# Labbeti/conette-audio-captioning

Hardware: AMD Instinct MI355X
Metric: clips_per_sec (higher is better)
Workload: dtype bf16; 1 GPU; B=64/GPU x 10 s @ 32 kHz clips, ConvNeXt encoder + beam-3 KV-cached decode (min 3 / max 20 tokens, V=5631), synthetic seeded checkpoint; batch_per_gpu=64, global_batch=64, beam_size=3, parallelism=dp1, world_size_observed=1, allreduce_of_ones=1, decode_group=2, decode_streams=2, encode_streams=1, input_batches_rotated=4

## Files before the change

conette-audio-captioning_amd/csrc/api.hip:

```cpp
#include <math.h>
#include <stdarg.h>
#include <stdlib.h>

#include <string>
#include <unordered_map>
#include <vector>

#include "ctx.h"
#include <algorithm>
#include "mlp_rc2.h"
#include "mlp_rs.h"
#include "mlp_rs16.h"
#include "mlp_sp.h"
#include "down_fused.h"

static thread_local char g_err[512] = "";

void cn_set_error(const char* fmt, ...) {
  va_list ap;
  va_start(ap, fmt);
  vsnprintf(g_err, sizeof(g_err), fmt, ap);
  va_end(ap);
}

extern "C" const char* conette_last_error(void) { return g_err; }

struct CnProfRec {
  int cls;
  hipEvent_t start, stop;
};
struct CnRuntime {
  std::vector<CnProfRec> recs;
  std::vector<hipEvent_t> free_ev;
  int open_cls = -1;
  hipEvent_t open_start = nullptr;
};

static hipEvent_t rt_event(CnRuntime* rt) {
  if (!rt->free_ev.empty()) {
    hipEvent_t e = rt->free_ev.back();
    rt->free_ev.pop_back();
    return e;
  }
  hipEvent_t e = nullptr;
  (void)hipEventCreate(&e);
  return e;
}

void cn_prof_begin(conette_ctx* ctx, int cls, hipStream_t s) {
  CnRuntime* rt = ctx->rt;
  rt->open_cls = cls;
  rt->open_start = rt_event(rt);
  (void)hipEventRecord(rt->open_start, s);
}
void cn_prof_end(conette_ctx* ctx, int cls, hipStream_t s) {
  CnRuntime* rt = ctx->rt;
  if (rt->open_cls != cls || !rt->open_start) return;
  hipEvent_t stop = rt_event(rt);
  (void)hipEventRecord(stop, s);
  rt->recs.push_back(CnProfRec{cls, rt->open_start, stop});
  rt->open_cls = -1;
  rt->open_start = nullptr;
}
// ... 150 lines not shown
    const float* src = find(name, n);
    if (n < 0) n = 0;
    float* dst = (float*)alloc((size_t)n * 4);
    if (src) hipLaunchKernelGGL((pk_copy<float>), dim3(256), dim3(256), 0, 0, src, dst, (size_t)n);
    return dst;
  }
  const void* operand(const std::string& name, int64_t total, int64_t first, int64_t n) {
    const float* src = find(name, total);
    void* dst = alloc((size_t)n * ctx->esize);
    if (src) {
      copy_operand(src + first, dst, (size_t)n);
    }
    return dst;
  }
  void copy_operand(const float* src, void* dst, size_t n) {
    if (ctx->esize == 2) CN_H16_CALL(ctx, hipLaunchKernelGGL((pk_copy<HT>), dim3(256), dim3(256), 0, 0, src, (HT*)dst, n));
    else if (ctx->sp16) hipLaunchKernelGGL((pk_copy<sp16_t>), dim3(256), dim3(256), 0, 0, src, (sp16_t*)dst, n);
    else hipLaunchKernelGGL((pk_copy<float>), dim3(256), dim3(256), 0, 0, src, (float*)dst, n);
  }
};

extern "C" int conette_create(const conette_config* cfg, int32_t n_tensors, const char* const* names,
                              const void* const* tensors, const int64_t* numel, conette_ctx** out) {
  if (!cfg || !names || !tensors || !numel || !out || n_tensors <= 0) {
    cn_set_error("create: bad argument");
    return CN_ERR_ARG;
  }
  if (cfg->precision != CONETTE_PREC_F32 && cfg->precision != CONETTE_PREC_BF16 && cfg->precision != CONETTE_PREC_F16X2 &&
      cfg->precision != CONETTE_PREC_F16) {
    cn_set_error(cfg->precision == 3 ? "create: precision 3 (the experimental fp8 mode of ABI 2) was withdrawn in ABI 3: e4m3 operands cost the "
                                       "frame embeddings 4 %% whatever the scaling (profiles/r06_notes.md section 3)"
                                     : "create: unknown precision %d", cfg->precision);
    return CN_ERR_ARG;
  }
  if (cfg->n_layers < 1 || cfg->n_layers > CN_MAX_LAYERS || cfg->d_model != 256 || cfg->nhead != 8 ||
      cfg->d_ff % 32 != 0 || cfg->vocab_size < 4) {
    cn_set_error("create: unsupported decoder geometry (d_model=%d nhead=%d layers=%d d_ff=%d)", cfg->d_model,
                 cfg->nhead, cfg->n_layers, cfg->d_ff);
    return CN_ERR_ARG;
  }
  conette_ctx* ctx = new conette_ctx();
  memset(ctx, 0, sizeof(*ctx));
  ctx->cfg = *cfg;
  ctx->rt = new CnRuntime();
  ctx->esize = (cfg->precision == CONETTE_PREC_BF16 || cfg->precision == CONETTE_PREC_F16) ? 2 : 4;
  ctx->f16 = cfg->precision == CONETTE_PREC_F16 ? 1 : 0;
  ctx->sp16 = cfg->precision == CONETTE_PREC_F16X2 ? 1 : 0;
  {
    int dev = 0, n_cu = 0;
    if (hipGetDevice(&dev) != hipSuccess || hipDeviceGetAttribute(&n_cu, hipDeviceAttributeMultiprocessorCount, dev) != hipSuccess ||
        n_cu <= 0)
      n_cu = 256;
    ctx->n_cu = n_cu;
  }
  size_t total = (1 << 20) + (size_t)CN_N_BINS * CN_N_MELS * 4;
  for (int i = 0; i < n_tensors; ++i) total += cn_align((size_t)numel[i] * 4) + 256;
  if (cfg->precision == CONETTE_PREC_F16X2) {
    total += 8u << 20;
    total += (size_t)cfg->n_layers * ((size_t)12 * 131072 + (size_t)(cfg->d_ff / 256 + 1) * 4 * 131072 + 4096);
  }
  ctx->arena_bytes = total;
  hipError_t e = hipMalloc((void**)&ctx->arena, total);
  if (e != hipSuccess) {
    cn_set_error("create: hipMalloc(%zu) -> %s", total, hipGetErrorString(e));
    delete ctx->rt;
    delete ctx;
    return CN_ERR_HIP;
  }
  Builder B;
  B.ctx = ctx;
  B.tensors = tensors;
  B.numel = numel;
  for (int i = 0; i < n_tensors; ++i) B.index[names[i]] = i;
  const int d = cfg->d_model, V = cfg->vocab_size, dff = cfg->d_ff;
  const std::string E = "preprocessor.encoder.";
  bool has_encoder = false;
  for (int i = 0; i < n_tensors && !has_encoder; ++i) has_encoder = strncmp(names[i], E.c_str(), E.size()) == 0;
  ctx->no_encoder = has_encoder ? 0 : 1;

  if (has_encoder) {
  {
    const float* cr = B.find(E + "spectrogram_extractor.stft.conv_real.weight", (int64_t)CN_N_BINS * CN_N_FFT);
    float* win = (float*)B.alloc(CN_N_FFT * 4);
    if (cr) hipMemcpy(win, cr, CN_N_FFT * 4, hipMemcpyDeviceToDevice);
    ctx->window = win;
    const float* ci = B.find(E + "spectrogram_extractor.stft.conv_imag.weight", (int64_t)CN_N_BINS * CN_N_FFT);
    if (cr && ci && B.err == CN_OK) {
      const int rows[5] = {1, 7, 100, 333, 512};
      std::vector<float> hw(CN_N_FFT), hr(CN_N_FFT), hi(CN_N_FFT);
      hipMemcpy(hw.data(), cr, CN_N_FFT * 4, hipMemcpyDeviceToHost);
      float wmax = 0.f;
      for (float v : hw) wmax = fmaxf(wmax, fabsf(v));
      double worst = 0.0;
      for (int k : rows) {
        hipMemcpy(hr.data(), cr + (size_t)k * CN_N_FFT, CN_N_FFT * 4, hipMemcpyDeviceToHost);
        hipMemcpy(hi.data(), ci + (size_t)k * CN_N_FFT, CN_N_FFT * 4, hipMemcpyDeviceToHost);
        for (int n = 0; n < CN_N_FFT; n += 13) {
          const double a = -2.0 * M_PI * (double)((long)k * n % CN_N_FFT) / CN_N_FFT;
          worst = fmax(worst, fabs(hr[n] - hw[n] * cos(a)));
          worst = fmax(worst, fabs(hi[n] - hw[n] * sin(a)));
        }
      }
      if (!(wmax > 0.f) || worst > 1e-4 * wmax) {
        cn_set_error("create: spectrogram_extractor.stft.conv_real / conv_imag are not a windowed DFT (max deviation %.3g of "
                     "window peak %.3g): the FFT frontend cannot reproduce this checkpoint", worst, (double)wmax);
        B.err = CN_ERR_WEIGHT;
// ... 389 lines not shown
```

conette-audio-captioning_amd/csrc/ctx.h:

```cpp
#pragma once
#include "../../include/conette_hip.h"
#include "common.h"

#define CN_N_MELS 224
#define CN_N_FFT 1024
#define CN_HOP 320
#define CN_N_BINS 513
#define CN_N_TAGS 527
#define CN_FEAT 768
#define CN_MAX_LAYERS 12

static const int CN_DEPTHS[4] = {3, 3, 9, 3};
static const int CN_DIMS[4] = {96, 192, 384, 768};

struct CnBlockW {
  const float* dw_w;
  const unsigned* dw_wp;
  const float* dw_b;
  const float* ln_w;
  const float* ln_b;
  const void* w1;
  const float* b1;
  const void* w2;
  const float* b2;
// ... 21 lines not shown
  const float* ca_out_b;
  const void* ff1_w;
  const float* ff1_b;
  const void* ff2_w;
  const float* ff2_b;
  const float *n1w, *n1b, *n2w, *n2b, *n3w, *n3b;
  const void* blk_w;
  const void* ffn_w;
  const float* blk_p;
};

struct CnRuntime;

struct conette_ctx {
  conette_config cfg;
  CnRuntime* rt;
  void* dec_graphs;
  uint32_t prof_mask;
  int dec_unfused;
  int esize;
  int sp16;
  int f16;
  int no_encoder;
  const float* window;
  const float2* tw512;
  const float2* tw1024;
  const int* band;
  int mel_rows;
  const float* melC;
  const float* bn_scale;
  const float* bn_shift;
  const float* stem_w;
  const float* stem_b;
  const float* stem_ln_w;
  const float* stem_ln_b;
  CnBlockW blocks[18];
  CnDownW down[3];
  const float* norm_w;
  const float* norm_b;
  const void* head_w;
  const float* head_b;
  const void* proj_w;
  const float* proj_b;
  const void* kv_w;
  const float* kv_b;
  CnLayerW layers[CN_MAX_LAYERS];
  const float* emb;
  const float* pe;
  int pe_len;
  const void* cls_w;
  const float* cls_b;
  int n_cu;
  int enc_reserved_cus;
  int forcing_stepwise;
  char* arena;
  size_t arena_bytes;
  size_t arena_used;
};

void cn_prof_begin(conette_ctx* ctx, int cls, hipStream_t s);
void cn_prof_end(conette_ctx* ctx, int cls, hipStream_t s);
struct CnProfScope {
  conette_ctx* ctx;
  int cls;
  hipStream_t s;
  CnProfScope(conette_ctx* c, int k, hipStream_t st) : ctx(c), cls(k), s(st) {
    if (ctx->prof_mask & (1u << cls)) cn_prof_begin(ctx, cls, s);
  }
  ~CnProfScope() {
    if (ctx->prof_mask & (1u << cls)) cn_prof_end(ctx, cls, s);
  }
};

int cn_frontend(conette_ctx* ctx, const float* wave, int B, int L, float* out, hipStream_t s);

#define CN_BY_PRECISION(ctx, ...)                                                          \
  do {                                                                                     \
    switch ((ctx)->cfg.precision) {                                                        \
      case CONETTE_PREC_BF16: { typedef bf16_t OT; return __VA_ARGS__; }                   \
      case CONETTE_PREC_F16: { typedef half_t OT; return __VA_ARGS__; }                    \
      case CONETTE_PREC_F16X2: { typedef sp16_t OT; return __VA_ARGS__; }                  \
      default: { typedef float OT; return __VA_ARGS__; }                                   \
    }                                                                                      \
  } while (0)
#define CN_H16_CALL(ctx, ...)                          \
  do {                                                 \
    if ((ctx)->f16) { typedef half_t HT; __VA_ARGS__; } \
    else { typedef bf16_t HT; __VA_ARGS__; }            \
  } while (0)
```

conette-audio-captioning_amd/csrc/encoder.hip:

```cpp
#include <stddef.h>

#include "ctx.h"
#include <type_traits>

__device__ int g_cn_nonfinite;
__device__ __forceinline__ void cn_watch_stat(float v) {
  if (!(__builtin_fabsf(v) <= 3.0e38f)) atomicAdd(&g_cn_nonfinite, 1);
}

#include "gemm2.h"
#include "mlp_rc2.h"
#include "mlp_rs.h"
#include "mlp_rs16.h"
#include "mlp_sp.h"
#include "down_fused.h"

#ifndef CN_DW_DOT2
#define CN_DW_DOT2 1
#endif

template <int P, typename XT>
__global__ __launch_bounds__(256) void cn_stem_kernel(const float* __restrict__ in, int F, int H0, long n_pos,
                                                      const float* __restrict__ w ,
                                                      const float* __restrict__ bias, const float* __restrict__ ln_w,
                                                      const float* __restrict__ ln_b, XT* __restrict__ out) {
  __shared__ __attribute__((aligned(16))) float s_w[16 * 96];
  __shared__ __attribute__((aligned(16))) float s_o[P * 64 * 96];
  for (int i = threadIdx.x; i < 16 * 96; i += 256) s_w[i] = w[i];
  __syncthreads();
  const int q = threadIdx.x & 3, lp = threadIdx.x >> 2;
  const long pos0 = (long)blockIdx.x * (64 * P);
  float xin[P][16];
#pragma unroll
  for (int u = 0; u < P; ++u) {
    const long pos = pos0 + 64 * u + lp;
    const long p = pos < n_pos ? pos : n_pos - 1;
    const int wq = (int)(p % 56);
    const long t = p / 56;
    const int h = (int)(t % H0);
    const int b = (int)(t / H0);
#pragma unroll
    for (int i = 0; i < 4; ++i) {
      const int r = 4 * h - 4 + i;
      f32x4 v = {0.f, 0.f, 0.f, 0.f};
      if (r >= 0 && r < F) v = *(const f32x4*)(in + ((size_t)b * F + r) * CN_N_MELS + 4 * wq);
      xin[u][4 * i] = v[0], xin[u][4 * i + 1] = v[1], xin[u][4 * i + 2] = v[2], xin[u][4 * i + 3] = v[3];
    }
  }
  f32x4 acc[P][6];
#pragma unroll
  for (int j = 0; j < 6; ++j) {
    const f32x4 b4 = *(const f32x4*)(bias + q * 24 + 4 * j);
#pragma unroll
    for (int u = 0; u < P; ++u) acc[u][j] = b4;
  }
#pragma unroll
  for (int i = 0; i < 16; ++i)
#pragma unroll
    for (int j = 0; j < 6; ++j) {
      const f32x4 w4 = *(const f32x4*)(s_w + i * 96 + q * 24 + 4 * j);
#pragma unroll
      for (int u = 0; u < P; ++u) acc[u][j] += xin[u][i] * w4;
    }
#pragma unroll
// ... 910 lines not shown
    const int C = CN_DIMS[st], H = g.H[st], W = g.W[st];
    const long P = (long)B * H * W;
    if (st > 0) {
      const int Cp = CN_DIMS[st - 1], Hp = g.H[st - 1], Wp = g.W[st - 1];
      const long n_in = (long)B * Hp * Wp;
      const CnDownW& dw = ctx->down[st - 1];
      CnProfScope ps(ctx, CONETTE_PROF_DOWNSAMPLE, s);
      bool fused_down = false;
      if constexpr (CnIsH16<T>::value) if (Cp <= 192 && dw.fused != nullptr) {
        XT* xo = xc == wsx ? (XT*)ws.h : wsx;
        const int nb = ctx->n_cu - ctx->enc_reserved_cus;
        if (Cp == 96) CN_TRY((cn_launch_down_fused<96, 8, T, XT>(xc, B, Hp, Wp, dw.fused, xo, nb, s)));
        else CN_TRY((cn_launch_down_fused_ring<192, 4, 4, 3, T, XT>(xc, B, Hp, Wp, dw.fused, xo, nb, s)));
        xc = xo;
        if (taps) CN_TRY(tap_copy(taps->down[st], xc, (size_t)P * C, s));
        fused_down = true;
      }
      if (!fused_down) {
      const int ppb = Cp == 96 ? 32 : 16;
      const dim3 pg((unsigned)((n_in + ppb - 1) / ppb));
      if (Cp == 96)
        hipLaunchKernelGGL((cn_ln_patchify_kernel<T, XT, 96>), pg, dim3(256), 0, s, xc, Hp, Wp, n_in, dw.ln_w, dw.ln_b, y);
      else if (Cp == 192)
        hipLaunchKernelGGL((cn_ln_patchify_kernel<T, XT, 192>), pg, dim3(256), 0, s, xc, Hp, Wp, n_in, dw.ln_w, dw.ln_b, y);
      else
        hipLaunchKernelGGL((cn_ln_patchify_kernel<T, XT, 384>), pg, dim3(256), 0, s, xc, Hp, Wp, n_in, dw.ln_w, dw.ln_b, y);
      CN_LAUNCH_CHECK();
      EpiBiasAct<XT, ACT_NONE> epi{dw.bias, wsx, C, ACT_NONE};
      CN_TRY(cn_mm(y, 4 * Cp, (const T*)dw.w, 4 * Cp, (int)P, C, 4 * Cp, epi, s));
      xc = wsx;
      if (taps) CN_TRY(tap_copy(taps->down[st], xc, (size_t)P * C, s));
      }
    }
    for (int b = 0; b < CN_DEPTHS[st]; ++b, ++blk) {
      const CnBlockW& bw = ctx->blocks[blk];
      {
        CnProfScope ps(ctx, CONETTE_PROF_DWCONV_LN, s);
        CN_TRY((dwconv_dispatch<T, XT>(C, xc, B, H, W, bw, y, s)));
      }
      bool fused = false;
      if constexpr (std::is_same<T, sp16_t>::value) {
        if (bw.mlp_sp != nullptr && C <= 192) {
          CnProfScope ps(ctx, CONETTE_PROF_PW1_GEMM, s);
          const int nb = ctx->n_cu - ctx->enc_reserved_cus;
          if (C == 96) CN_TRY((cn_launch_mlp_sp_ring<96, CN_SP_NW96, CN_SP_NST96>(y, bw.mlp_sp, xc, (int)P, nb, s)));
          else CN_TRY((cn_launch_mlp_sp_ring<192, 8, 3>(y, bw.mlp_sp, xc, (int)P, nb, s)));
          fused = true;
        }
      }
      if constexpr (CnIsH16<T>::value) if (!fused) {
        if (bw.mlp_stream != nullptr && C <= 384) {
          CnProfScope ps(ctx, CONETTE_PROF_PW1_GEMM, s);
          const T* wsm = (const T*)bw.mlp_stream;
          if (C == 96) CN_TRY((cn_launch_mlp_rc2_resident<96, 12, 1>(y, wsm, xc, (int)P, ctx->n_cu - ctx->enc_reserved_cus, s)));
          else if (C == 192) CN_TRY((cn_launch_mlp_rc2_ring<192, 8, CN_RC2_NCK(192), CN_RC2_NCK(192) == 2 ? 3 : 5>(y, wsm, xc, (int)P, ctx->n_cu - ctx->enc_reserved_cus, s)));
#ifdef CN_NO_RS
          else CN_TRY((cn_launch_mlp_rc2_ring<384, 4, 1, 3>(y, wsm, xc, (int)P, ctx->n_cu - ctx->enc_reserved_cus, s)));
#else
          else if constexpr (sizeof(XT) == 2 && CN_RS16) CN_TRY((cn_launch_mlp_rs16<384, 4, 3, CN_RS_PRIO>(y, wsm, xc, (int)P, ctx->n_cu - ctx->enc_reserved_cus, s)));
          else CN_TRY((cn_launch_mlp_rs<384, 4, 3, CN_RS_PRIO>(y, wsm, xc, (int)P, ctx->n_cu - ctx->enc_reserved_cus, s)));
#endif
          fused = true;
        }
      }
      if (!fused) {
        {
          CnProfScope ps(ctx, CONETTE_PROF_PW1_GEMM, s);
#ifdef CN_G2_NOACT
          constexpr int kAct = ACT_NONE;
#else
          constexpr int kAct = CnGeluAct<T>::value;
#endif
          EpiBiasAct<T, kAct> e1{bw.b1, hbuf, 4 * C, kAct};
          CN_TRY(cn_mm(y, C, (const T*)bw.w1, C, (int)P, 4 * C, C, e1, s));
        }
        {
          CnProfScope ps(ctx, CONETTE_PROF_PW2_GEMM, s);
          EpiResidT<XT> e2{bw.b2, bw.scale, xc, xc, C};
          CN_TRY(cn_mm(hbuf, 4 * C, (const T*)bw.w2, 4 * C, (int)P, C, 4 * C, e2, s));
        }
      }
      if (taps && b == 0) CN_TRY(tap_copy(taps->stage_block0[st], xc, (size_t)P * C, s));
      if (taps && taps->struct_bytes >= offsetof(conette_encode_taps, block) + (size_t)(blk + 1) * sizeof(float*))
        CN_TRY(tap_copy(taps->block[blk], xc, (size_t)P * C, s));
    }
    if (taps) CN_TRY(tap_copy(taps->stage[st], xc, (size_t)P * C, s));
  }
  const int Tn = g.H[3];
  CnProfScope ps_heads(ctx, CONETTE_PROF_HEADS, s);
  hipLaunchKernelGGL((cn_frame_mean_kernel<T, XT>), dim3((unsigned)(B * Tn)), dim3(256), 0, s, xc, g.W[3], CN_FEAT,
                     frame_embs, (T*)nullptr);
  CN_LAUNCH_CHECK();
  if (clip_probs) {
    hipLaunchKernelGGL((cn_clip_pool_ln_kernel<T>), dim3((unsigned)B), dim3(256), 0, s, frame_embs, Tn, ctx->norm_w,
                       ctx->norm_b, (T*)ws.clip_t);
    CN_LAUNCH_CHECK();
    EpiBiasAct<float> eh{ctx->head_b, clip_probs, CN_N_TAGS, ACT_SIGMOID};
    CN_TRY(cn_mm((const T*)ws.clip_t, CN_FEAT, (const T*)ctx->head_w, CN_FEAT, B, CN_N_TAGS, CN_FEAT, eh, s));
  }
  return CN_OK;
}

extern "C" int conette_encode_nonfinite(conette_ctx* ctx, void* stream, int32_t* count) {
  if (!ctx || !count) {
    cn_set_error("encode_nonfinite: bad argument");
    return CN_ERR_ARG;
  }
// ... 65 lines not shown
```

conette-audio-captioning_amd/csrc/mlp_rc2.h:

```cpp
#pragma once
#include "common.h"

template <int C, int NCK> struct Rc2Geom {
  static constexpr int KS1 = C / 16, NT2 = C / 32, NCH = C / 8;
  static constexpr int F1 = KS1 + 1, F2 = 2 * NT2;
  static constexpr int NSTEP = NCH / NCK;
  static constexpr int FRAGS = NCK * (F1 + F2);
  static constexpr int STEP_BYTES = FRAGS * 1024;
  static constexpr size_t STREAM_BYTES = (size_t)NSTEP * STEP_BYTES;
  static constexpr size_t TOTAL_BYTES = STREAM_BYTES + NT2 * 1024;
};
__host__ __device__ constexpr int cn_rc2_chan(int m) { return (m & 19) | ((m & 4) << 1) | ((m & 8) >> 1); }

__device__ __forceinline__ float cn_gelu_sig2(float x) {
  constexpr float L2E = 1.4426950408889634f;
  const float x2 = fminf(x * x, 64.0f);
  float p = fmaf(x2, 0.0007030350670982541f * L2E, -0.07401130190658815f * L2E);
  p = fmaf(p, x2, -1.5950157568571721f * L2E);
  const float e = __builtin_amdgcn_exp2f(x * p);
  return x * __builtin_amdgcn_rcpf(1.0f + e);
}

#if defined(CN_GELU_SIG2)
#define CN_MLP_XSCALE 1.0f
// ... 25 lines not shown
static __global__ void pk_mlp_rc2(const float* __restrict__ W1, const float* __restrict__ b1, const float* __restrict__ W2,
                           const float* __restrict__ b2, const float* __restrict__ scale, int C, int NCK,
                           HT* __restrict__ dst) {
  const int KS1 = C / 16, NT2 = C / 32, NCH = C / 8, F1 = KS1 + 1, F2 = 2 * NT2, FRAGS = NCK * (F1 + F2), NSTEP = NCH / NCK;
  const int u = blockIdx.x * blockDim.x + threadIdx.x;
  if (u >= (NSTEP * FRAGS + NT2) * 64) return;
  const int l = u & 63, q = (u >> 6) % FRAGS, st = (u >> 6) / FRAGS;
  const int r = l & 31, h = l >> 5;
  float v[8];
  if (st >= NSTEP) {
    const int c = 32 * q + cn_rc2_chan(r);
    const float b = scale[c] * b2[c];
    const float hi = (float)(HT)b;
#pragma unroll
    for (int i = 0; i < 8; ++i) v[i] = 0.f;
    if (h == 0) {
      v[0] = hi;
      v[1] = b - hi;
    }
  } else if (q < NCK * F1) {
    const int j = st * NCK + q / F1, s = q % F1;
    if (s < KS1) {
#pragma unroll
      for (int i = 0; i < 8; ++i) v[i] = CN_MLP_XSCALE * W1[(size_t)(32 * j + r) * C + 16 * s + 8 * h + i];
    } else {
      const float b = CN_MLP_XSCALE * b1[32 * j + r];
      const float hi = (float)(HT)b;
#pragma unroll
      for (int i = 0; i < 8; ++i) v[i] = 0.f;
      if (h == 0) {
        v[0] = hi;
        v[1] = b - hi;
      }
    }
  } else {
    const int q2 = q - NCK * F1;
    const int j = st * NCK + q2 / F2, s = (q2 % F2) / NT2, t = (q2 % F2) % NT2;
    const int c = 32 * t + cn_rc2_chan(r);
    const float sc = scale[c];
#pragma unroll
    for (int i = 0; i < 8; ++i) v[i] = sc * W2[(size_t)c * (4 * C) + 32 * j + 16 * s + 8 * (i >> 2) + 4 * h + (i & 3)];
  }
#pragma unroll
  for (int i = 0; i < 8; ++i) dst[(size_t)u * 8 + i] = (HT)v[i];
}

#define CN_RC2_NCK(C) ((C) == 192 ? 2 : 1)

#define CN_SG_VALU 0x002
#define CN_SG_MFMA 0x008
#define CN_SG_DSR 0x100


template <int C, int NCK, typename HT = bf16_t, typename XT = float> struct Rc2Wave {
  typedef Rc2Geom<C, NCK> G;
  typedef cn_h8<HT> hx8;
  static constexpr int KS1 = G::KS1, NT2 = G::NT2, F1 = G::F1, F2 = G::F2;
  static constexpr int NV = 88;

  static __device__ __forceinline__ hx8 frag(const char* wc, int f) { return *(const hx8*)(wc + f * 1024); }
  static __device__ __forceinline__ f32x16 mma(hx8 a, hx8 b, f32x16 c) { return cn_mma32(a, b, c); }
  static __device__ __forceinline__ hx8 gelu8(const f32x16& X, int o) {
    float g[8];
#pragma unroll
    for (int i = 0; i < 8; ++i) g[i] = cn_gelu_mlp<HT>(X[o + i]);
    return cn_sat8<HT>(cn_pack8<HT>(g[0], g[1], g[2], g[3], g[4], g[5], g[6], g[7]));
  }
  static __device__ __forceinline__ f32x16 zero16() {
    f32x16 z;
#pragma unroll
    for (int i = 0; i < 16; ++i) z[i] = 0.f;
    return z;
  }

  static constexpr int PRE = 4;
  static constexpr int NM = NCK * (F1 + F2), R = PRE + 1;
  struct State {
    hx8 F[R];
    f32x16 X[NCK];
    float g[NCK][16];
    hx8 H[NCK][2];
  };
  static constexpr int gelu_at(int i, int e) {
    if (NCK == 2) return i == 0 ? F1 + 1 + e * (F1 - 1) / 16 : 2 * F1 + e * F2 / 16;
    return e < 8 ? F1 - 1 : F1 + (e - 8) * NT2 / 8;
  }
  template <int Q, int I, int E>
  static __device__ __forceinline__ void gelu_slices(State& st) {
#if defined(CN_RC2_GELU_PK) && defined(CN_GELU_SIG2)
    if constexpr ((E & 1) == 0 && gelu_at(I, E) == Q) {
      const f32x2 r = cn_gelu_sig2_pk(f32x2{st.X[I][E], st.X[I][E + 1]});
      st.g[I][E] = r[0];
      st.g[I][E + 1] = r[1];
    }
    if constexpr (gelu_at(I, E & ~1) == Q) {
#else
    if constexpr (gelu_at(I, E) == Q) {
      st.g[I][E] = cn_gelu_mlp<HT>(st.X[I][E]);
#endif
      if constexpr ((E & 7) == 7) {
        constexpr int o = E - 7;
        st.H[I][E >> 3] = cn_sat8<HT>(cn_pack8<HT>(st.g[I][o], st.g[I][o + 1], st.g[I][o + 2], st.g[I][o + 3],
                                                   st.g[I][o + 4], st.g[I][o + 5], st.g[I][o + 6], st.g[I][o + 7]));
      }
    }
    if constexpr (E + 1 < 16) gelu_slices<Q, I, E + 1>(st);
    else if constexpr (I + 1 < NCK) gelu_slices<Q, I + 1, 0>(st);
  }
  template <int Q>
  static __device__ __forceinline__ void mstep(const char* wc, const hx8 (&fy)[KS1], const hx8 ones, f32x16 (&O)[NT2],
                                               State& st) {
    if constexpr (Q + PRE < NM) st.F[(Q + PRE) % R] = frag(wc, Q + PRE);
    if constexpr (Q < NCK * F1) {
      constexpr int i = Q / F1, s = Q % F1;
      if constexpr (s == 0) st.X[i] = zero16();
      if constexpr (s < KS1) st.X[i] = mma(st.F[Q % R], fy[s], st.X[i]);
      else st.X[i] = mma(st.F[Q % R], ones, st.X[i]);
    } else {
      constexpr int q2 = Q - NCK * F1, i = q2 / F2, k = (q2 % F2) / NT2, t = q2 % NT2;
      O[t] = mma(st.F[Q % R], st.H[i][k], O[t]);
    }
    gelu_slices<Q, 0, 0>(st);
    __builtin_amdgcn_sched_barrier(0);
    if constexpr (Q + 1 < NM) mstep<Q + 1>(wc, fy, ones, O, st);
  }
  template <int Q>
  static __device__ __forceinline__ void prefetch(const char* wc, State& st) {
    st.F[Q % R] = frag(wc, Q);
    if constexpr (Q + 1 < PRE) prefetch<Q + 1>(wc, st);
  }
  static __device__ __forceinline__ void step(const char* wc, const hx8 (&fy)[KS1], const hx8 ones, f32x16 (&O)[NT2]) {
    State st;
    prefetch<0>(wc, st);
    __builtin_amdgcn_sched_barrier(0);
    mstep<0>(wc, fy, ones, O, st);
  }


  static __device__ __forceinline__ void load_y(const HT* __restrict__ Y, int m0, int lane, hx8 (&fy)[KS1]) {
    const HT* base = Y + (size_t)m0 * C;
    const int voff = (lane & 31) * C + 8 * (lane >> 5);
#pragma unroll
    for (int s = 0; s < KS1; ++s) fy[s] = *(const hx8*)(base + voff + 16 * s);
  }

  static __device__ __forceinline__ void init_o(const XT* __restrict__ X, const char* __restrict__ bbf, const hx8 ones, int m0,
                                                int lane, f32x16 (&O)[NT2]) {
    const XT* base = X + (size_t)m0 * C;
    const int voff = (lane & 31) * C + 8 * (lane >> 5);
    hx8 fb[NT2];
    if constexpr (sizeof(XT) == 2) {
      cn_h8<XT> v[NT2][2];
#pragma unroll
      for (int t = 0; t < NT2; ++t) {
        v[t][0] = *(const cn_h8<XT>*)(base + voff + 32 * t);
        v[t][1] = *(const cn_h8<XT>*)(base + voff + 32 * t + 16);
      }
#pragma unroll
// ... 28 lines not shown
#pragma unroll
        for (int o = 0; o < 2; ++o)
          *(cn_h8<XT>*)(base + voff + 32 * t + 16 * o) = cn_pack8<XT>(O[t][8 * o], O[t][8 * o + 1], O[t][8 * o + 2], O[t][8 * o + 3],
                                                                      O[t][8 * o + 4], O[t][8 * o + 5], O[t][8 * o + 6], O[t][8 * o + 7]);
      } else {
#pragma unroll
        for (int q = 0; q < 4; ++q)
          *(f32x4*)(base + voff + 32 * t + 16 * (q >> 1) + 4 * (q & 1)) = f32x4{O[t][4 * q], O[t][4 * q + 1], O[t][4 * q + 2], O[t][4 * q + 3]};
      }
    }
  }
};

template <int C> struct Rc2IoCl {
  static constexpr int NT2 = C / 32;
  static __device__ __forceinline__ void init_o(const float* __restrict__ X, int m0, int lane, f32x16 (&O)[NT2]) {
    const int voff = 4 * (lane >> 5) * C + (lane & 31);
#pragma unroll
    for (int r = 0; r < 16; ++r) {
      const float* row = X + (size_t)(m0 + (r & 3) + 8 * (r >> 2)) * C;
#pragma unroll
      for (int t = 0; t < NT2; ++t) O[t][r] = row[voff + 32 * t];
    }
  }
  static __device__ __forceinline__ void store_o(float* __restrict__ X, const float* __restrict__ bbv, int m0, int M, int lane,
                                                 const f32x16 (&O)[NT2]) {
    const int voff = 4 * (lane >> 5) * C + (lane & 31);
    const int plim = M - m0 - 4 * (lane >> 5);
    float bb[NT2];
#pragma unroll
    for (int t = 0; t < NT2; ++t) bb[t] = bbv[32 * t + (lane & 31)];
#pragma unroll
    for (int r = 0; r < 16; ++r) {
      float* row = X + (size_t)(m0 + (r & 3) + 8 * (r >> 2)) * C;
      if ((r & 3) + 8 * (r >> 2) < plim) {
#pragma unroll
        for (int t = 0; t < NT2; ++t) row[voff + 32 * t] = O[t][r] + bb[t];
      }
    }
  }
};

static inline int cn_rc2_grid(int n_tiles, int waves_per_block, int max_blocks) {
  const int block_tiles = cn_cdiv(n_tiles, waves_per_block);
  if (max_blocks < 1) max_blocks = 1;
  const int rounds = cn_cdiv(block_tiles, max_blocks);
  return cn_cdiv(block_tiles, rounds);
}

template <int C, int NW, int NCK, typename HT = bf16_t, int ABL = 0, typename XT = float>
__global__ __launch_bounds__(NW * 64) void cn_mlp_rc2_resident_kernel(const HT* __restrict__ Y, const HT* __restrict__ WS,
                                                                      XT* __restrict__ X, int M) {
  typedef Rc2Geom<C, NCK> G;
  typedef Rc2Wave<C, NCK, HT, XT> W;
  typedef cn_h8<HT> hx8;
  extern __shared__ __attribute__((aligned(16))) char smem[];
  const int tid = threadIdx.x, lane = tid & 63;
  const int wave = __builtin_amdgcn_readfirstlane(tid >> 6);
  constexpr int TOTAL = G::NSTEP * G::FRAGS;
  for (int i = wave; i < TOTAL; i += NW)
    __builtin_amdgcn_global_load_lds((const __attribute__((address_space(1))) void*)((const char*)WS + (size_t)i * 1024 + lane * 16),
                                     (__attribute__((address_space(3))) void*)(smem + i * 1024), 16, 0, 0);
  const char* bbf = (const char*)WS + G::STREAM_BYTES + lane * 16;
  const int n_tiles = (M + 31) >> 5;
  const int t_lo = (int)((long)blockIdx.x * n_tiles / gridDim.x), t_hi = (int)((long)(blockIdx.x + 1) * n_tiles / gridDim.x);
  hx8 ones;
#pragma unroll
  for (int i = 0; i < 8; ++i) ones[i] = (HT)((lane < 32 && i < 2) ? 1.0f : 0.0f);
  hx8 fy[G::KS1];
  int tile = t_lo + wave;
  if (tile < t_hi) W::load_y(Y, tile * 32, lane, fy);
  asm volatile("s_waitcnt vmcnt(0)" ::: "memory");
  __syncthreads();
  const char* wl = smem + lane * 16;
  for (; tile < t_hi; tile += NW) {
    f32x16 O[G::NT2];
    if constexpr (ABL & 1) {
#pragma unroll
      for (int t = 0; t < G::NT2; ++t) O[t] = W::zero16();
    } else {
      W::init_o(X, bbf, ones, tile * 32, lane, O);
    }
#pragma unroll 1
    for (int j = 0; j < G::NSTEP; ++j) W::step(wl + j * G::STEP_BYTES, fy, ones, O);
    if constexpr (!(ABL & 8))
      if (tile + NW < t_hi) W::load_y(Y, (tile + NW) * 32, lane, fy);
    if constexpr (ABL & 2) {
      if (O[0][0] == 12345.678f) W::store_o(X, tile * 32, M, lane, O);
    } else {
      W::store_o(X, tile * 32, M, lane, O);
    }
  }
}

template <int C, int NW, int NCK, int ABL = 0, typename HT, typename XT>
static int cn_launch_mlp_rc2_resident(const HT* Y, const HT* WS, XT* X, int M, int n_blocks, hipStream_t s) {
  constexpr int SMEM = (int)Rc2Geom<C, NCK>::STREAM_BYTES;
  static_assert(SMEM <= 160 * 1024, "resident variant: the weight stream must fit in LDS");
  CN_TRY(cn_configure_lds((const void*)cn_mlp_rc2_resident_kernel<C, NW, NCK, HT, ABL, XT>, SMEM));
  const int grid = cn_rc2_grid((M + 31) / 32, NW, n_blocks);
  hipLaunchKernelGGL((cn_mlp_rc2_resident_kernel<C, NW, NCK, HT, ABL, XT>), dim3((unsigned)grid), dim3(NW * 64), SMEM, s, Y, WS, X, M);
  CN_LAUNCH_CHECK();
  return CN_OK;
}

template <int C, int NW, int NCK, int NST, int PROF = 0, typename HT = bf16_t, typename XT = float>
__global__ __launch_bounds__(NW * 64) void cn_mlp_rc2_ring_kernel(const HT* __restrict__ Y, const HT* __restrict__ WS,
                                                                  XT* __restrict__ X, int M, unsigned long long* prof = nullptr) {
  unsigned long long tacc[5] = {0, 0, 0, 0, 0}, tprev = 0, nstep = 0;
  auto stamp = [&](int i) {
    if constexpr (PROF) {
      const unsigned long long t = clock64();
      tacc[i] += t - tprev;
      tprev = t;
    }
  };
  if constexpr (PROF) tprev = clock64();
  typedef Rc2Geom<C, NCK> G;
  typedef Rc2Wave<C, NCK, HT, XT> W;
  typedef cn_h8<HT> hx8;
  constexpr int FR = G::FRAGS, SB = G::STEP_BYTES;
  constexpr int DPW_LO = FR / NW, N_HI = FR % NW;
  extern __shared__ __attribute__((aligned(16))) char smem[];
  const int tid = threadIdx.x, lane = tid & 63;
  const int wave = __builtin_amdgcn_readfirstlane(tid >> 6);
  const char* bbf = (const char*)WS + G::STREAM_BYTES + lane * 16;

  const int n_tiles = (M + 31) >> 5;
  const int t_lo = (int)((long)blockIdx.x * n_tiles / gridDim.x), t_hi = (int)((long)(blockIdx.x + 1) * n_tiles / gridDim.x);
  const int max_it = (t_hi - t_lo + NW - 1) / NW;

  const unsigned voff = lane * 16;
  const unsigned lds0 = cn_lds_addr(smem);
  auto stage = [&](int g) {
    const char* src = (const char*)WS + (size_t)(g % G::NSTEP) * SB;
    const unsigned dst = lds0 + (unsigned)((g % NST) * SB);
#pragma unroll
    for (int i = 0; i < DPW_LO + 1; ++i) {
      const int piece = wave + i * NW;
      if (i < DPW_LO || wave < N_HI) cn_dma16_s(src + piece * 1024, voff, dst + piece * 1024);
    }
  };
  hx8 ones;
#pragma unroll
  for (int i = 0; i < 8; ++i) ones[i] = (HT)((lane < 32 && i < 2) ? 1.0f : 0.0f);

#pragma unroll
  for (int g = 0; g < NST - 1; ++g) stage(g);
  hx8 fy[G::KS1];
  if (t_lo + wave < t_hi) W::load_y(Y, (t_lo + wave) * 32, lane, fy);
  const char* wl = smem + lane * 16;
  int g = 0;
  for (int it = 0; it < max_it; ++it) {
    const int tile = t_lo + wave + it * NW;
    const bool valid = tile < t_hi;
    f32x16 O[G::NT2];
    if (valid) W::init_o(X, bbf, ones, tile * 32, lane, O);
    {
      __builtin_amdgcn_s_waitcnt(0x0F70);
    }
    for (int j = 0; j < G::NSTEP; ++j, ++g) {
      stamp(4);
      if (N_HI > 0 && wave < N_HI) asm volatile("s_waitcnt vmcnt(%0)" ::"n"((NST - 2) * (DPW_LO + 1)) : "memory");
      else asm volatile("s_waitcnt vmcnt(%0)" ::"n"((NST - 2) * DPW_LO) : "memory");
      stamp(0);
      __builtin_amdgcn_s_barrier();
      stamp(1);
      stage(g + NST - 1);
      stamp(2);
      if (valid) W::step(wl + (g % NST) * SB, fy, ones, O);
      stamp(3);
      if constexpr (PROF) nstep += valid;
    }
    if (tile + NW < t_hi) W::load_y(Y, (tile + NW) * 32, lane, fy);
    if (valid) W::store_o(X, tile * 32, M, lane, O);
  }
  asm volatile("s_waitcnt vmcnt(0)" ::: "memory");
  if constexpr (PROF) {
    if (lane == 0 && prof) {
#pragma unroll
      for (int i = 0; i < 5; ++i) atomicAdd(prof + i, tacc[i]);
      atomicAdd(prof + 5, nstep);
    }
  }
}

template <int C, int NW, int NCK, int NST, int PROF = 0, typename HT, typename XT>
static int cn_launch_mlp_rc2_ring(const HT* Y, const HT* WS, XT* X, int M, int n_blocks, hipStream_t s,
                                  unsigned long long* prof = nullptr) {
  constexpr int SMEM = NST * Rc2Geom<C, NCK>::STEP_BYTES;
  static_assert(SMEM <= 160 * 1024, "ring must fit in LDS");
  CN_TRY(cn_configure_lds((const void*)cn_mlp_rc2_ring_kernel<C, NW, NCK, NST, PROF, HT, XT>, SMEM));
  const int grid = cn_rc2_grid((M + 31) / 32, NW, n_blocks);
  hipLaunchKernelGGL((cn_mlp_rc2_ring_kernel<C, NW, NCK, NST, PROF, HT, XT>), dim3((unsigned)grid), dim3(NW * 64), SMEM, s, Y, WS, X, M, prof);
  CN_LAUNCH_CHECK();
  return CN_OK;
}
```

Before: 13170 clips/s.

## Add software-pipelined resident MLP kernel for stage-0 ConvNeXt blocks

Adds a new resident-weight MLP kernel for C=96 that software-pipelines the two GEMMs across hidden chunks. It prefetches LDS weight fragments several slots ahead and overlaps the GELU of one chunk with the PW1 MMA of the next and the PW2 MMA of the previous, using double-buffered accumulators. The kernel is enabled by default and can be turned off through an environment variable. It also adds ablation template flags (skip init/store, alternate GELU) to the existing rc2 kernels, which default to off. The aim is to hide LDS latency and GELU ALU time behind MFMA work, at the cost of higher register pressure.

```diff
diff --git a/conette-audio-captioning_amd/csrc/api.hip b/conette-audio-captioning_amd/csrc/api.hip
--- a/conette-audio-captioning_amd/csrc/api.hip
+++ b/conette-audio-captioning_amd/csrc/api.hip
@@ -9,6 +9,7 @@
 #include "ctx.h"
 #include <algorithm>
 #include "mlp_rc2.h"
+#include "mlp_rc2p.h"
 #include "mlp_rs.h"
 #include "mlp_rs16.h"
 #include "mlp_sp.h"
@@ -265,6 +266,10 @@
         n_cu <= 0)
       n_cu = 256;
     ctx->n_cu = n_cu;
+  }
+  {
+    const char* e = getenv("CN_RC2_PIPE");
+    ctx->rc2_pipe = e ? (atoi(e) != 0) : CN_RC2_PIPE;
   }
   size_t total = (1 << 20) + (size_t)CN_N_BINS * CN_N_MELS * 4;
   for (int i = 0; i < n_tensors; ++i) total += cn_align((size_t)numel[i] * 4) + 256;
diff --git a/conette-audio-captioning_amd/csrc/ctx.h b/conette-audio-captioning_amd/csrc/ctx.h
--- a/conette-audio-captioning_amd/csrc/ctx.h
+++ b/conette-audio-captioning_amd/csrc/ctx.h
@@ -97,6 +97,7 @@
   const float* cls_b;
   int n_cu;
   int enc_reserved_cus;
+  int rc2_pipe;
   int forcing_stepwise;
   char* arena;
   size_t arena_bytes;
diff --git a/conette-audio-captioning_amd/csrc/encoder.hip b/conette-audio-captioning_amd/csrc/encoder.hip
--- a/conette-audio-captioning_amd/csrc/encoder.hip
+++ b/conette-audio-captioning_amd/csrc/encoder.hip
@@ -10,6 +10,7 @@
 
 #include "gemm2.h"
 #include "mlp_rc2.h"
+#include "mlp_rc2p.h"
 #include "mlp_rs.h"
 #include "mlp_rs16.h"
 #include "mlp_sp.h"
@@ -1026,7 +1027,8 @@
         if (bw.mlp_stream != nullptr && C <= 384) {
           CnProfScope ps(ctx, CONETTE_PROF_PW1_GEMM, s);
           const T* wsm = (const T*)bw.mlp_stream;
-          if (C == 96) CN_TRY((cn_launch_mlp_rc2_resident<96, 12, 1>(y, wsm, xc, (int)P, ctx->n_cu - ctx->enc_reserved_cus, s)));
+          if (C == 96 && ctx->rc2_pipe) CN_TRY((cn_launch_mlp_rc2p_resident<96, 12>(y, wsm, xc, (int)P, ctx->n_cu - ctx->enc_reserved_cus, s)));
+          else if (C == 96) CN_TRY((cn_launch_mlp_rc2_resident<96, 12, 1>(y, wsm, xc, (int)P, ctx->n_cu - ctx->enc_reserved_cus, s)));
           else if (C == 192) CN_TRY((cn_launch_mlp_rc2_ring<192, 8, CN_RC2_NCK(192), CN_RC2_NCK(192) == 2 ? 3 : 5>(y, wsm, xc, (int)P, ctx->n_cu - ctx->enc_reserved_cus, s)));
 #ifdef CN_NO_RS
           else CN_TRY((cn_launch_mlp_rc2_ring<384, 4, 1, 3>(y, wsm, xc, (int)P, ctx->n_cu - ctx->enc_reserved_cus, s)));
diff --git a/conette-audio-captioning_amd/csrc/mlp_rc2.h b/conette-audio-captioning_amd/csrc/mlp_rc2.h
--- a/conette-audio-captioning_amd/csrc/mlp_rc2.h
+++ b/conette-audio-captioning_amd/csrc/mlp_rc2.h
@@ -101,11 +101,22 @@
 #define CN_SG_DSR 0x100
 
 
-template <int C, int NCK, typename HT = bf16_t, typename XT = float> struct Rc2Wave {
+template <int C, int NCK, typename HT = bf16_t, typename XT = float, int AG = 0> struct Rc2Wave {
   typedef Rc2Geom<C, NCK> G;
   typedef cn_h8<HT> hx8;
   static constexpr int KS1 = G::KS1, NT2 = G::NT2, F1 = G::F1, F2 = G::F2;
   static constexpr int NV = 88;
+
+  template <int E>
+  static __device__ __forceinline__ void gelu_elem(const f32x16& X, float (&g)[16], hx8& h) {
+    if constexpr (AG == 0) g[E] = cn_gelu_mlp<HT>(X[E]);
+    else if constexpr (AG == 1) g[E] = X[E];
+    if constexpr ((E & 7) == 7) {
+      constexpr int o = E - 7;
+      if constexpr (AG == 2) h = __builtin_bit_cast(hx8, f32x4{X[o], X[o + 1], X[o + 2], X[o + 3]});
+      else h = cn_sat8<HT>(cn_pack8<HT>(g[o], g[o + 1], g[o + 2], g[o + 3], g[o + 4], g[o + 5], g[o + 6], g[o + 7]));
+    }
+  }
 
   static __device__ __forceinline__ hx8 frag(const char* wc, int f) { return *(const hx8*)(wc + f * 1024); }
   static __device__ __forceinline__ f32x16 mma(hx8 a, hx8 b, f32x16 c) { return cn_mma32(a, b, c); }
@@ -142,17 +153,14 @@
       st.g[I][E] = r[0];
       st.g[I][E + 1] = r[1];
     }
-    if constexpr (gelu_at(I, E & ~1) == Q) {
+    if constexpr (gelu_at(I, E & ~1) == Q && (E & 7) == 7) {
+      constexpr int o = E - 7;
+      st.H[I][E >> 3] = cn_sat8<HT>(cn_pack8<HT>(st.g[I][o], st.g[I][o + 1], st.g[I][o + 2], st.g[I][o + 3],
+                                                 st.g[I][o + 4], st.g[I][o + 5], st.g[I][o + 6], st.g[I][o + 7]));
+    }
 #else
-    if constexpr (gelu_at(I, E) == Q) {
-      st.g[I][E] = cn_gelu_mlp<HT>(st.X[I][E]);
+    if constexpr (gelu_at(I, E) == Q) gelu_elem<E>(st.X[I], st.g[I], st.H[I][E >> 3]);
 #endif
-      if constexpr ((E & 7) == 7) {
-        constexpr int o = E - 7;
-        st.H[I][E >> 3] = cn_sat8<HT>(cn_pack8<HT>(st.g[I][o], st.g[I][o + 1], st.g[I][o + 2], st.g[I][o + 3],
-                                                   st.g[I][o + 4], st.g[I][o + 5], st.g[I][o + 6], st.g[I][o + 7]));
-      }
-    }
     if constexpr (E + 1 < 16) gelu_slices<Q, I, E + 1>(st);
     else if constexpr (I + 1 < NCK) gelu_slices<Q, I + 1, 0>(st);
   }
@@ -287,7 +295,7 @@
 __global__ __launch_bounds__(NW * 64) void cn_mlp_rc2_resident_kernel(const HT* __restrict__ Y, const HT* __restrict__ WS,
                                                                       XT* __restrict__ X, int M) {
   typedef Rc2Geom<C, NCK> G;
-  typedef Rc2Wave<C, NCK, HT, XT> W;
+  typedef Rc2Wave<C, NCK, HT, XT, (ABL >> 4) & 3> W;
   typedef cn_h8<HT> hx8;
   extern __shared__ __attribute__((aligned(16))) char smem[];
   const int tid = threadIdx.x, lane = tid & 63;
@@ -339,7 +347,7 @@
   return CN_OK;
 }
 
-template <int C, int NW, int NCK, int NST, int PROF = 0, typename HT = bf16_t, typename XT = float>
+template <int C, int NW, int NCK, int NST, int PROF = 0, typename HT = bf16_t, typename XT = float, int ABL = 0>
 __global__ __launch_bounds__(NW * 64) void cn_mlp_rc2_ring_kernel(const HT* __restrict__ Y, const HT* __restrict__ WS,
                                                                   XT* __restrict__ X, int M, unsigned long long* prof = nullptr) {
   unsigned long long tacc[5] = {0, 0, 0, 0, 0}, tprev = 0, nstep = 0;
@@ -352,7 +360,7 @@
   };
   if constexpr (PROF) tprev = clock64();
   typedef Rc2Geom<C, NCK> G;
-  typedef Rc2Wave<C, NCK, HT, XT> W;
+  typedef Rc2Wave<C, NCK, HT, XT, (ABL >> 4) & 3> W;
   typedef cn_h8<HT> hx8;
   constexpr int FR = G::FRAGS, SB = G::STEP_BYTES;
   constexpr int DPW_LO = FR / NW, N_HI = FR % NW;
@@ -368,6 +376,7 @@
   const unsigned voff = lane * 16;
   const unsigned lds0 = cn_lds_addr(smem);
   auto stage = [&](int g) {
+    if constexpr (ABL & 4) if (g >= NST - 1) return;
     const char* src = (const char*)WS + (size_t)(g % G::NSTEP) * SB;
     const unsigned dst = lds0 + (unsigned)((g % NST) * SB);
 #pragma unroll
@@ -390,7 +399,10 @@
     const int tile = t_lo + wave + it * NW;
     const bool valid = tile < t_hi;
     f32x16 O[G::NT2];
-    if (valid) W::init_o(X, bbf, ones, tile * 32, lane, O);
+    if constexpr (ABL & 1) {
+#pragma unroll
+      for (int t = 0; t < G::NT2; ++t) O[t] = W::zero16();
+    } else if (valid) W::init_o(X, bbf, ones, tile * 32, lane, O);
     {
       __builtin_amdgcn_s_waitcnt(0x0F70);
     }
@@ -408,7 +420,9 @@
       if constexpr (PROF) nstep += valid;
     }
     if (tile + NW < t_hi) W::load_y(Y, (tile + NW) * 32, lane, fy);
-    if (valid) W::store_o(X, tile * 32, M, lane, O);
+    if constexpr (ABL & 2) {
+      if (valid && O[0][0] == 12345.678f) W::store_o(X, tile * 32, M, lane, O);
+    } else if (valid) W::store_o(X, tile * 32, M, lane, O);
   }
   asm volatile("s_waitcnt vmcnt(0)" ::: "memory");
   if constexpr (PROF) {
@@ -420,14 +434,14 @@
   }
 }
 
-template <int C, int NW, int NCK, int NST, int PROF = 0, typename HT, typename XT>
+template <int C, int NW, int NCK, int NST, int PROF = 0, int ABL = 0, typename HT, typename XT>
 static int cn_launch_mlp_rc2_ring(const HT* Y, const HT* WS, XT* X, int M, int n_blocks, hipStream_t s,
                                   unsigned long long* prof = nullptr) {
   constexpr int SMEM = NST * Rc2Geom<C, NCK>::STEP_BYTES;
   static_assert(SMEM <= 160 * 1024, "ring must fit in LDS");
-  CN_TRY(cn_configure_lds((const void*)cn_mlp_rc2_ring_kernel<C, NW, NCK, NST, PROF, HT, XT>, SMEM));
+  CN_TRY(cn_configure_lds((const void*)cn_mlp_rc2_ring_kernel<C, NW, NCK, NST, PROF, HT, XT, ABL>, SMEM));
   const int grid = cn_rc2_grid((M + 31) / 32, NW, n_blocks);
-  hipLaunchKernelGGL((cn_mlp_rc2_ring_kernel<C, NW, NCK, NST, PROF, HT, XT>), dim3((unsigned)grid), dim3(NW * 64), SMEM, s, Y, WS, X, M, prof);
+  hipLaunchKernelGGL((cn_mlp_rc2_ring_kernel<C, NW, NCK, NST, PROF, HT, XT, ABL>), dim3((unsigned)grid), dim3(NW * 64), SMEM, s, Y, WS, X, M, prof);
   CN_LAUNCH_CHECK();
   return CN_OK;
 }
diff --git a/conette-audio-captioning_amd/csrc/mlp_rc2p.h b/conette-audio-captioning_amd/csrc/mlp_rc2p.h
--- /dev/null
+++ b/conette-audio-captioning_amd/csrc/mlp_rc2p.h
@@ -0,0 +1,142 @@
+#pragma once
+#include "mlp_rc2.h"
+
+#ifndef CN_RC2_PIPE
+#define CN_RC2_PIPE 1
+#endif
+
+template <int C, typename HT = bf16_t, typename XT = float, int AG = 0> struct Rc2Pipe {
+  typedef Rc2Wave<C, 1, HT, XT, AG> W;
+  typedef Rc2Geom<C, 1> G;
+  typedef cn_h8<HT> hx8;
+  static constexpr int KS1 = G::KS1, NT2 = G::NT2, F1 = G::F1, F2 = G::F2, NCH = G::NCH, SB = G::STEP_BYTES;
+  static constexpr int NQ = F1 + F2;
+  static_assert(F1 == F2 + 1 && NCH % 2 == 0, "slot table");
+  static constexpr int PRE = 4, R = PRE + 1;
+
+  static constexpr int m1_of(int q) { return q < 2 ? q : (q & 1) ? (q + 1) / 2 : -1; }
+  static constexpr int m2_of(int q) { return q < 2 || (q & 1) ? -1 : (q - 2) / 2; }
+  static constexpr int gelu_at(int e) { return e * NQ / 16; }
+
+  struct State {
+    hx8 F[R];
+    f32x16 X[2];
+    float g[16];
+    hx8 H[2][2];
+  };
+
+  template <int Q, bool A1, bool A2>
+  static __device__ __forceinline__ void fetch(const char* w1, const char* w2, State& st) {
+    if constexpr (m1_of(Q) >= 0) {
+      if constexpr (A1) st.F[Q % R] = W::frag(w1, m1_of(Q));
+    } else {
+      if constexpr (A2) st.F[Q % R] = W::frag(w2, m2_of(Q));
+    }
+  }
+  template <int Q, int E, int P>
+  static __device__ __forceinline__ void gelu_slices(State& st) {
+    if constexpr (gelu_at(E) == Q) W::template gelu_elem<E>(st.X[P], st.g, st.H[P][E >> 3]);
+    if constexpr (E + 1 < 16) gelu_slices<Q, E + 1, P>(st);
+  }
+  template <int Q, int P, bool A1, bool AGL, bool A2>
+  static __device__ __forceinline__ void slot(const char* w1, const char* w2, const hx8 (&fy)[KS1], const hx8 ones,
+                                              f32x16 (&O)[NT2], State& st) {
+    if constexpr (Q + PRE < NQ) fetch<Q + PRE, A1, A2>(w1, w2, st);
+    constexpr int k1 = m1_of(Q), i2 = m2_of(Q);
+    if constexpr (k1 >= 0 && A1) {
+      constexpr int N = P ^ 1;
+      if constexpr (k1 == 0) st.X[N] = W::zero16();
+      if constexpr (k1 < KS1) st.X[N] = W::mma(st.F[Q % R], fy[k1], st.X[N]);
+      else st.X[N] = W::mma(st.F[Q % R], ones, st.X[N]);
+    }
+    if constexpr (i2 >= 0 && A2) {
+      constexpr int k = i2 / NT2, t = i2 % NT2;
+      O[t] = W::mma(st.F[Q % R], st.H[P ^ 1][k], O[t]);
+    }
+    if constexpr (AGL) gelu_slices<Q, 0, P>(st);
+    __builtin_amdgcn_sched_barrier(0);
+    if constexpr (Q + 1 < NQ) slot<Q + 1, P, A1, AGL, A2>(w1, w2, fy, ones, O, st);
+  }
+  template <int Q, bool A1, bool A2>
+  static __device__ __forceinline__ void prefetch(const char* w1, const char* w2, State& st) {
+    fetch<Q, A1, A2>(w1, w2, st);
+    if constexpr (Q + 1 < PRE) prefetch<Q + 1, A1, A2>(w1, w2, st);
+  }
+  template <int P, bool A1, bool AGL, bool A2>
+  static __device__ __forceinline__ void step(const char* w1, const char* w2, const hx8 (&fy)[KS1], const hx8 ones,
+                                              f32x16 (&O)[NT2], State& st) {
+    prefetch<0, A1, A2>(w1, w2, st);
+    __builtin_amdgcn_sched_barrier(0);
+    slot<0, P, A1, AGL, A2>(w1, w2, fy, ones, O, st);
+  }
+
+  static __device__ __forceinline__ void tile(const char* wl, const hx8 (&fy)[KS1], const hx8 ones, f32x16 (&O)[NT2]) {
+    State st;
+    const char* w2d = wl + F1 * 1024;
+    step<1, true, false, false>(wl, nullptr, fy, ones, O, st);
+    step<0, true, true, false>(wl + SB, nullptr, fy, ones, O, st);
+#pragma unroll 1
+    for (int s = 1; s < NCH - 1; s += 2) {
+      step<1, true, true, true>(wl + (s + 1) * SB, w2d + (s - 1) * SB, fy, ones, O, st);
+      step<0, true, true, true>(wl + (s + 2) * SB, w2d + s * SB, fy, ones, O, st);
+    }
+    step<1, false, true, true>(nullptr, w2d + (NCH - 2) * SB, fy, ones, O, st);
+    step<0, false, false, true>(nullptr, w2d + (NCH - 1) * SB, fy, ones, O, st);
+  }
+};
+
+template <int C, int NW, typename HT = bf16_t, int ABL = 0, typename XT = float>
+__global__ __launch_bounds__(NW * 64) void cn_mlp_rc2p_resident_kernel(const HT* __restrict__ Y, const HT* __restrict__ WS,
+                                                                       XT* __restrict__ X, int M) {
+  typedef Rc2Geom<C, 1> G;
+  typedef Rc2Pipe<C, HT, XT, (ABL >> 4) & 3> PW;
+  typedef typename PW::W W;
+  typedef cn_h8<HT> hx8;
+  extern __shared__ __attribute__((aligned(16))) char smem[];
+  const int tid = threadIdx.x, lane = tid & 63;
+  const int wave = __builtin_amdgcn_readfirstlane(tid >> 6);
+  constexpr int TOTAL = G::NSTEP * G::FRAGS;
+  for (int i = wave; i < TOTAL; i += NW)
+    __builtin_amdgcn_global_load_lds((const __attribute__((address_space(1))) void*)((const char*)WS + (size_t)i * 1024 + lane * 16),
+                                     (__attribute__((address_space(3))) void*)(smem + i * 1024), 16, 0, 0);
+  const char* bbf = (const char*)WS + G::STREAM_BYTES + lane * 16;
+  const int n_tiles = (M + 31) >> 5;
+  const int t_lo = (int)((long)blockIdx.x * n_tiles / gridDim.x), t_hi = (int)((long)(blockIdx.x + 1) * n_tiles / gridDim.x);
+  hx8 ones;
+#pragma unroll
+  for (int i = 0; i < 8; ++i) ones[i] = (HT)((lane < 32 && i < 2) ? 1.0f : 0.0f);
+  hx8 fy[G::KS1];
+  int tile = t_lo + wave;
+  if (tile < t_hi) W::load_y(Y, tile * 32, lane, fy);
+  asm volatile("s_waitcnt vmcnt(0)" ::: "memory");
+  __syncthreads();
+  const char* wl = smem + lane * 16;
+  for (; tile < t_hi; tile += NW) {
+    f32x16 O[G::NT2];
+    if constexpr (ABL & 1) {
+#pragma unroll
+      for (int t = 0; t < G::NT2; ++t) O[t] = W::zero16();
+    } else {
+      W::init_o(X, bbf, ones, tile * 32, lane, O);
+    }
+    PW::tile(wl, fy, ones, O);
+    if constexpr (!(ABL & 8))
+      if (tile + NW < t_hi) W::load_y(Y, (tile + NW) * 32, lane, fy);
+    if constexpr (ABL & 2) {
+      if (O[0][0] == 12345.678f) W::store_o(X, tile * 32, M, lane, O);
+    } else {
+      W::store_o(X, tile * 32, M, lane, O);
+    }
+  }
+}
+
+template <int C, int NW, int ABL = 0, typename HT, typename XT>
+static int cn_launch_mlp_rc2p_resident(const HT* Y, const HT* WS, XT* X, int M, int n_blocks, hipStream_t s) {
+  constexpr int SMEM = (int)Rc2Geom<C, 1>::STREAM_BYTES;
+  static_assert(SMEM <= 160 * 1024, "resident variant: the weight stream must fit in LDS");
+  CN_TRY(cn_configure_lds((const void*)cn_mlp_rc2p_resident_kernel<C, NW, HT, ABL, XT>, SMEM));
+  const int grid = cn_rc2_grid((M + 31) / 32, NW, n_blocks);
+  hipLaunchKernelGGL((cn_mlp_rc2p_resident_kernel<C, NW, HT, ABL, XT>), dim3((unsigned)grid), dim3(NW * 64), SMEM, s, Y, WS, X, M);
+  CN_LAUNCH_CHECK();
+  return CN_OK;
+}
```

Result: no change. 13130 clips/s, median of 3 (-0.3%).
